# KinWaiCheuk/nnAudio

Hardware: AMD Instinct MI355X
Metric: spectrogram frames/sec (higher is better)
Workload: dtype f32; 1 GPU; STFT n_fft=2048 hop=512 hann, B=64 x 10 s @ 44.1 kHz, Magnitude (configs[1]); global_batch=64, precision=fp32 FFT per frame (VALU), err ~2e-7 of peak, parallelism=batch-sharded x1, no data-path collective

## Files before the change

nnaudio_amd/csrc/fft_core.h:

```cpp
#pragma once

#if defined(__HIPCC__)
#define FFT_HD __host__ __device__ __forceinline__
#else
#define FFT_HD inline
#endif

namespace fftcore {

typedef float cf __attribute__((ext_vector_type(2)));

FFT_HD cf cmul(cf a, cf w) { return cf{a.x * w.x - a.y * w.y, a.x * w.y + a.y * w.x}; }
FFT_HD cf mul_mi(cf a) { return cf{a.y, -a.x}; }

FFT_HD void dft2(cf &a, cf &b) {
  const cf t = a - b;
  a = a + b;
  b = t;
}

FFT_HD void dft4(cf (&v)[4]) {
  const cf s02 = v[0] + v[2], d02 = v[0] - v[2];
  const cf s13 = v[1] + v[3], d13 = mul_mi(v[1] - v[3]);
  v[0] = s02 + s13;
  v[1] = d02 + d13;
  v[2] = s02 - s13;
  v[3] = d02 - d13;
}

FFT_HD void dft8(cf (&v)[8]) {
  cf e[4] = {v[0], v[2], v[4], v[6]}, o[4] = {v[1], v[3], v[5], v[7]};
  dft4(e);
  dft4(o);
  constexpr float h = 0.70710678118654752f;
  const cf t1 = cf{(o[1].x + o[1].y) * h, (o[1].y - o[1].x) * h};
  const cf t2 = mul_mi(o[2]);
  const cf t3 = cf{(o[3].y - o[3].x) * h, -(o[3].x + o[3].y) * h};
  v[0] = e[0] + o[0];
  v[4] = e[0] - o[0];
  v[1] = e[1] + t1;
  v[5] = e[1] - t1;
  v[2] = e[2] + t2;
  v[6] = e[2] - t2;
  v[3] = e[3] + t3;
  v[7] = e[3] - t3;
}

FFT_HD void dft16(cf (&v)[16]) {
  cf e[8], o[8];
#pragma unroll
  for (int i = 0; i < 8; ++i) {
    e[i] = v[2 * i];
    o[i] = v[2 * i + 1];
  }
  dft8(e);
  dft8(o);
  constexpr float c1 = 0.92387953251128674f, s1 = 0.38268343236508977f;
  constexpr float h = 0.70710678118654752f;
  const cf w[8] = {cf{1.f, 0.f}, cf{c1, -s1}, cf{h, -h}, cf{s1, -c1}, cf{0.f, -1.f}, cf{-s1, -c1}, cf{-h, -h}, cf{-c1, -s1}};
#pragma unroll
  for (int k = 0; k < 8; ++k) {
    cf t;
    if (k == 0)
      t = o[0];
    else if (k == 4)
      t = mul_mi(o[4]);
    else if (k == 2)
      t = cf{(o[2].x + o[2].y) * h, (o[2].y - o[2].x) * h};
    else if (k == 6)
      t = cf{(o[6].y - o[6].x) * h, -(o[6].x + o[6].y) * h};
    else
      t = cmul(o[k], w[k]);
    v[k] = e[k] + t;
    v[k + 8] = e[k] - t;
  }
}

template <int R>
FFT_HD void dft(cf (&v)[R]) {
  static_assert(R == 2 || R == 4 || R == 8 || R == 16, "radix");
  if constexpr (R == 2) dft2(v[0], v[1]);
  if constexpr (R == 4) dft4(v);
  if constexpr (R == 8) dft8(v);
  if constexpr (R == 16) dft16(v);
}

FFT_HD int pad(int o) { return o + (o >> 4); }
template <int M>
constexpr int padded_size() {
  return M + (M >> 4) + 1;
}

template <int M>
struct Radix;
template <>
struct Radix<1024> {
  static constexpr int n = 3, r0 = 16, r1 = 16, r2 = 4, r3 = 1;
};
template <>
struct Radix<512> {
  static constexpr int n = 3, r0 = 8, r1 = 8, r2 = 8, r3 = 1;
};
template <>
struct Radix<256> {
  static constexpr int n = 4, r0 = 4, r1 = 4, r2 = 4, r3 = 4;
};
template <int M, int PASS>
constexpr int radix_of() {
  return PASS == 0 ? Radix<M>::r0 : PASS == 1 ? Radix<M>::r1 : PASS == 2 ? Radix<M>::r2 : Radix<M>::r3;
}
template <int M, int PASS>
constexpr int ns_of() {
  int ns = 1;
  if (PASS > 0) ns *= Radix<M>::r0;
  if (PASS > 1) ns *= Radix<M>::r1;
  if (PASS > 2) ns *= Radix<M>::r2;
  return ns;
}
template <int M, int PASS>
constexpr int tw_count() {
  return PASS == 0 ? 0 : (M / 64 / radix_of<M, PASS>()) * (radix_of<M, PASS>() - 1);
}
template <int M>
constexpr int tw_total() {
  return tw_count<M, 1>() + tw_count<M, 2>() + (Radix<M>::n > 3 ? tw_count<M, 3>() : 0);
}
template <int M, int PASS>
constexpr int tw_offset() {
  return PASS <= 1 ? 0 : PASS == 2 ? tw_count<M, 1>() : tw_count<M, 1>() + tw_count<M, 2>();
}

template <int M, int PASS>
FFT_HD float tw_turns(int lane, int idx) {
  constexpr int R = radix_of<M, PASS>(), NS = ns_of<M, PASS>();
  const int q = idx / (R - 1), r = idx % (R - 1) + 1;
  const int k = (lane + 64 * q) & (NS - 1);
  return -(float)(r * k) / (float)(NS * R);
}

template <int M, int PASS, typename Tw, typename Store>
FFT_HD void stockham_pass(cf (&x)[M / 64], int lane, Tw &&twf, Store &&store) {
  constexpr int P = M / 64, R = radix_of<M, PASS>(), NS = ns_of<M, PASS>(), Q = P / R;
  static_assert(P % R == 0, "a lane holds whole butterflies");
#pragma unroll
  for (int q = 0; q < Q; ++q) {
    cf v[R];
#pragma unroll
    for (int r = 0; r < R; ++r) v[r] = x[q + r * Q];
    if constexpr (NS > 1) {
#pragma unroll
      for (int r = 1; r < R; ++r) v[r] = cmul(v[r], twf(q, r));
    }
    dft<R>(v);
    const int j = lane + 64 * q, k = j & (NS - 1);
    const int base = (j - k) * R + k;
#pragma unroll
    for (int r = 0; r < R; ++r) {
      x[q + r * Q] = v[r];
      store(base + r * NS, v[r]);
    }
  }
}

FFT_HD cf real_post(cf zk, cf zm, cf wh) {
  const cf a = cf{zk.x + zm.x, zk.y - zm.y} * 0.5f;
  const cf b = cf{zk.x - zm.x, zk.y + zm.y};
  const cf wb = cmul(b, wh);
  return cf{a.x + wb.y, a.y - wb.x};
}

FFT_HD void real_post_pair(cf zk, cf zm, cf wh, cf &xk, cf &xm) {
  const cf a = cf{zk.x + zm.x, zk.y - zm.y} * 0.5f;
  const cf b = cf{zk.x - zm.x, zk.y + zm.y};
  const cf wb = cmul(b, wh);
  xk = cf{a.x + wb.y, a.y - wb.x};
  xm = cf{a.x - wb.y, -(a.y + wb.x)};
}

FFT_HD cf real_pre_conj(cf gk, cf gm, cf w) {
  const cf a = cf{gk.x + gm.x, gk.y - gm.y};
  const cf b = cf{gk.x - gm.x, gk.y + gm.y};
  const cf wb = cmul(b, w);
  return cf{a.x - wb.y, -(a.y + wb.x)};
}

}
```

Baseline: 414.9 million frames/s.

## Rewrite FFT butterflies with packed-f32 FMA inline asm and fused twiddles

Adds packed v_pk_add/v_pk_fma_f32 inline-asm butterfly primitives and restructures the radix-2/4/8/16 DFTs as a first butterfly stage followed by recursive twiddled butterflies. The first stage of each twiddled Stockham pass is folded into an FMA-based butterfly (b = 2a - s), which cuts instruction count on the VALU-bound FFT. The change is on by default via a macro and risks small numerical differences from the FMA reassociation, plus register pressure or scheduling constraints from the inline asm.

```diff
diff --git a/nnaudio_amd/csrc/fft_core.h b/nnaudio_amd/csrc/fft_core.h
--- a/nnaudio_amd/csrc/fft_core.h
+++ b/nnaudio_amd/csrc/fft_core.h
@@ -13,6 +13,181 @@
 FFT_HD cf cmul(cf a, cf w) { return cf{a.x * w.x - a.y * w.y, a.x * w.y + a.y * w.x}; }
 FFT_HD cf mul_mi(cf a) { return cf{a.y, -a.x}; }
 
+#ifndef MISPEC_FFT_PK
+#define MISPEC_FFT_PK 1
+#endif
+#if MISPEC_FFT_PK && defined(__HIP_DEVICE_COMPILE__)
+#define FFT_PK_ASM 1
+#else
+#define FFT_PK_ASM 0
+#endif
+
+FFT_HD cf fma2(cf a, cf b, cf c) { return cf{__builtin_fmaf(a.x, b.x, c.x), __builtin_fmaf(a.y, b.y, c.y)}; }
+
+FFT_HD void bf(cf &a, cf &b) {
+  const cf t = a - b;
+  a = a + b;
+  b = t;
+}
+
+FFT_HD void bf_mi(cf &a, cf &b) {
+#if FFT_PK_ASM
+  cf s, d;
+  asm("v_pk_add_f32 %0, %1, %2 op_sel:[0,1] op_sel_hi:[1,0] neg_hi:[0,1]" : "=v"(s) : "v"(a), "v"(b));
+  asm("v_pk_add_f32 %0, %1, %2 op_sel:[0,1] op_sel_hi:[1,0] neg_lo:[0,1]" : "=v"(d) : "v"(a), "v"(b));
+  a = s;
+  b = d;
+#else
+  const cf s = cf{a.x + b.y, a.y - b.x}, d = cf{a.x - b.y, a.y + b.x};
+  a = s;
+  b = d;
+#endif
+}
+
+FFT_HD void bf_w8(cf &a, cf &b) {
+  constexpr float h = 0.70710678118654752f;
+#if FFT_PK_ASM
+  const cf hh = cf{h, h};
+  cf u, s, d;
+  asm("v_pk_add_f32 %0, %1, %1 op_sel:[0,1] op_sel_hi:[1,0] neg_hi:[0,1]" : "=v"(u) : "v"(b));
+  asm("v_pk_fma_f32 %0, %1, %2, %3 op_sel_hi:[1,0,1]" : "=v"(s) : "v"(u), "s"(hh), "v"(a));
+  asm("v_pk_fma_f32 %0, %1, %2, %3 op_sel_hi:[1,0,1] neg_lo:[0,1,0] neg_hi:[0,1,0]" : "=v"(d) : "v"(u), "s"(hh), "v"(a));
+  a = s;
+  b = d;
+#else
+  const cf u = cf{b.x + b.y, b.y - b.x};
+  const cf s = fma2(u, cf{h, h}, a), d = fma2(u, cf{-h, -h}, a);
+  a = s;
+  b = d;
+#endif
+}
+
+FFT_HD void bf_w83(cf &a, cf &b) {
+  constexpr float h = 0.70710678118654752f;
+#if FFT_PK_ASM
+  const cf hh = cf{h, h};
+  cf u, s, d;
+  asm("v_pk_add_f32 %0, %1, %1 op_sel:[1,0] op_sel_hi:[0,1] neg_lo:[0,1] neg_hi:[1,1]" : "=v"(u) : "v"(b));
+  asm("v_pk_fma_f32 %0, %1, %2, %3 op_sel_hi:[1,0,1]" : "=v"(s) : "v"(u), "s"(hh), "v"(a));
+  asm("v_pk_fma_f32 %0, %1, %2, %3 op_sel_hi:[1,0,1] neg_lo:[0,1,0] neg_hi:[0,1,0]" : "=v"(d) : "v"(u), "s"(hh), "v"(a));
+  a = s;
+  b = d;
+#else
+  const cf u = cf{b.y - b.x, -b.x - b.y};
+  const cf s = fma2(u, cf{h, h}, a), d = fma2(u, cf{-h, -h}, a);
+  a = s;
+  b = d;
+#endif
+}
+
+template <bool SW = false>
+FFT_HD void bf_tw(cf &a, cf &b, cf w) {
+#if FFT_PK_ASM
+  cf t, s, d;
+  if constexpr (SW) {
+    asm("v_pk_fma_f32 %0, %1, %2, %3 op_sel_hi:[0,1,1]" : "=v"(t) : "v"(b), "s"(w), "v"(a));
+    asm("v_pk_fma_f32 %0, %1, %2, %3 op_sel:[1,1,0] op_sel_hi:[1,0,1] neg_lo:[0,1,0]" : "=v"(s) : "v"(b), "s"(w), "v"(t));
+  } else {
+    asm("v_pk_fma_f32 %0, %1, %2, %3 op_sel_hi:[0,1,1]" : "=v"(t) : "v"(b), "v"(w), "v"(a));
+    asm("v_pk_fma_f32 %0, %1, %2, %3 op_sel:[1,1,0] op_sel_hi:[1,0,1] neg_lo:[0,1,0]" : "=v"(s) : "v"(b), "v"(w), "v"(t));
+  }
+  asm("v_pk_fma_f32 %0, %1, 2.0, %2 op_sel_hi:[1,0,1] neg_lo:[0,0,1] neg_hi:[0,0,1]" : "=v"(d) : "v"(a), "v"(s));
+  a = s;
+  b = d;
+#else
+  const cf t = fma2(cf{b.x, b.x}, w, a);
+  const cf s = fma2(cf{b.y, b.y}, cf{-w.y, w.x}, t);
+  b = fma2(a, cf{2.f, 2.f}, -s);
+  a = s;
+#endif
+}
+
+FFT_HD cf cmul_pk(cf a, cf w) {
+#if FFT_PK_ASM
+  cf t, r;
+  asm("v_pk_mul_f32 %0, %1, %2 op_sel_hi:[0,1]" : "=v"(t) : "v"(a), "v"(w));
+  asm("v_pk_fma_f32 %0, %1, %2, %3 op_sel:[1,1,0] op_sel_hi:[1,0,1] neg_lo:[0,1,0]" : "=v"(r) : "v"(a), "v"(w), "v"(t));
+  return r;
+#else
+  const cf t = cf{a.x, a.x} * w;
+  return fma2(cf{a.y, a.y}, cf{-w.y, w.x}, t);
+#endif
+}
+
+#if MISPEC_FFT_PK
+template <int R>
+FFT_HD void dft_first(cf (&v)[R]) {
+#pragma unroll
+  for (int r = 0; r < R / 2; ++r) bf(v[r], v[r + R / 2]);
+}
+template <int R, typename Tw>
+FFT_HD void dft_first_tw(cf (&v)[R], Tw &&tw) {
+#pragma unroll
+  for (int r = 0; r < R / 2; ++r) {
+    if (r > 0) v[r] = cmul_pk(v[r], tw(r));
+    bf_tw(v[r], v[r + R / 2], tw(r + R / 2));
+  }
+}
+
+FFT_HD void dft_rest(cf (&v)[2]) {}
+
+FFT_HD void dft_rest(cf (&v)[4]) {
+  cf a = v[0], b = v[1], c = v[2], d = v[3];
+  bf(a, b);
+  bf_mi(c, d);
+  v[0] = a;
+  v[1] = c;
+  v[2] = b;
+  v[3] = d;
+}
+
+FFT_HD void dft_rest(cf (&v)[8]) {
+  cf e[4] = {v[0], v[2], v[4], v[6]}, o[4] = {v[1], v[3], v[5], v[7]};
+  dft_rest(e);
+  dft_rest(o);
+  bf(e[0], o[0]);
+  bf_w8(e[1], o[1]);
+  bf_mi(e[2], o[2]);
+  bf_w83(e[3], o[3]);
+#pragma unroll
+  for (int k = 0; k < 4; ++k) {
+    v[k] = e[k];
+    v[k + 4] = o[k];
+  }
+}
+
+FFT_HD void dft_rest(cf (&v)[16]) {
+  cf e[8], o[8];
+#pragma unroll
+  for (int i = 0; i < 8; ++i) {
+    e[i] = v[2 * i];
+    o[i] = v[2 * i + 1];
+  }
+  dft_rest(e);
+  dft_rest(o);
+  constexpr float c1 = 0.92387953251128674f, s1 = 0.38268343236508977f;
+  bf(e[0], o[0]);
+  bf_tw<true>(e[1], o[1], cf{c1, -s1});
+  bf_w8(e[2], o[2]);
+  bf_tw<true>(e[3], o[3], cf{s1, -c1});
+  bf_mi(e[4], o[4]);
+  bf_tw<true>(e[5], o[5], cf{-s1, -c1});
+  bf_w83(e[6], o[6]);
+  bf_tw<true>(e[7], o[7], cf{-c1, -s1});
+#pragma unroll
+  for (int k = 0; k < 8; ++k) {
+    v[k] = e[k];
+    v[k + 8] = o[k];
+  }
+}
+
+template <int R>
+FFT_HD void dft(cf (&v)[R]) {
+  static_assert(R == 2 || R == 4 || R == 8 || R == 16, "radix");
+  dft_first(v);
+  dft_rest(v);
+}
+#else
 FFT_HD void dft2(cf &a, cf &b) {
   const cf t = a - b;
   a = a + b;
@@ -85,6 +260,8 @@
   if constexpr (R == 16) dft16(v);
 }
 
+#endif
+
 FFT_HD int pad(int o) { return o + (o >> 4); }
 template <int M>
 constexpr int padded_size() {
@@ -147,11 +324,20 @@
     cf v[R];
 #pragma unroll
     for (int r = 0; r < R; ++r) v[r] = x[q + r * Q];
+#if MISPEC_FFT_PK
+    if constexpr (NS > 1) {
+      dft_first_tw(v, [&](int r) __attribute__((always_inline)) { return twf(q, r); });
+      dft_rest(v);
+    } else {
+      dft(v);
+    }
+#else
     if constexpr (NS > 1) {
 #pragma unroll
       for (int r = 1; r < R; ++r) v[r] = cmul(v[r], twf(q, r));
     }
     dft<R>(v);
+#endif
     const int j = lane + 64 * q, k = j & (NS - 1);
     const int base = (j - k) * R + k;
 #pragma unroll
```

Measured after the change: 418.9 million frames/s (median of 6 runs). About the same (+1.0%).
